# tky823/DNN-based_source_separation

Hardware: NVIDIA H100
Metric: audio-sec/s Conv-TasNet 2spk 4s@8kHz fwd+SI-SDR-PIT (higher is better)
Workload: dtype f32 via 3xFP16 split on wgmma (f16), fp32 accumulate

## Files before the change

dnn-based_source_separation_b200/csrc/ctn_wgmma.cu:

```cuda
#include "ctn_internal.h"
#include "ctn_wgmma_ptx.cuh"
#include "ctn_dw_math.cuh"
#include <cuda_fp16.h>
#include <stdlib.h>
#include <string.h>

int ctn_pw_simt(const PwArgs& a, int pro, int epi, cudaStream_t st);

namespace {

constexpr int TM = 128;
constexpr int KS = 32;
constexpr int NT = 128;
constexpr int THREADS = 256;
constexpr int CPW = 4;
constexpr int STAGES = 2;
constexpr int SMEM_HEADER = 1024;
constexpr int F16_MAX_ROWS = 2048;

template <int PRO, int EPI, bool F16>
__host__ __device__ constexpr bool chan_split() { return F16 && (PRO == PRO_DW || EPI == EPI_H); }
template <int PRO, int EPI, bool F16>
__host__ __device__ constexpr int tile_frames() { return chan_split<PRO, EPI, F16>() ? 64 : TM; }

struct TcArgs {
  PwArgs a;
  const float* wimg;
  const float* oscale;
  int n_tiles, k_slabs, t_tiles;
  int n_groups;
  int nt_per_cta;
};

template <int PRO>
__host__ __device__ constexpr int raw_q() { return PRO == PRO_DW ? 3 : PRO == PRO_RES ? 2 : 1; }
template <int PRO, int CPT>
struct Raw { float4 q[CPT][raw_q<PRO>()]; };

template <int PRO, int CPT>
__device__ __forceinline__ void load_raw(const PwArgs& a, int b, int c0, int tbase, int first, int step, bool interior, Raw<PRO, CPT>& r) {
#pragma unroll
  for (int j = 0; j < CPT; ++j) {
    const int c = c0 + j;
    if constexpr (PRO == PRO_DW) {
      const int cc = interior ? c : (c < a.K ? c : a.K - 1);
      const float* hr = a.A + ((size_t)b * a.K + cc) * a.pitch;
#pragma unroll
      for (int k = 0; k < 3; ++k) {
        int ts = first + k * step;
        if (!interior) ts = ts < 0 ? 0 : (ts > a.pitch - 4 ? a.pitch - 4 : ts);
        r.q[j][k] = __ldg(reinterpret_cast<const float4*>(hr + ts));
      }
    } else {
      const bool ok = c < a.K;
      r.q[j][0] = ok ? __ldg(reinterpret_cast<const float4*>(a.A + ((size_t)b * a.K + c) * a.pitch + tbase)) : make_float4(0.f, 0.f, 0.f, 0.f);
      if constexpr (PRO == PRO_RES)
        r.q[j][1] = ok ? __ldg(reinterpret_cast<const float4*>(a.res_r + ((size_t)b * a.res_Mt + c) * a.pitch + tbase))
                       : make_float4(0.f, 0.f, 0.f, 0.f);
    }
  }
}

template <int DCLS, bool INTERIOR, bool TRAIN, int CPT>
__device__ __forceinline__ void dw_form(const PwArgs& a, int b, int c0, int tbase, int first, int step, float2 mr1, float pslope,
                                        bool store_side, Raw<PRO_DW, CPT>& r, float4 (&v)[CPT], float2& dls, float2& dlss) {
  const float islope = TRAIN ? __ldg(a.dw_in_slope) : 0.f;
#pragma unroll
  for (int j = 0; j < CPT; ++j) {
    const int c = c0 + j;
    const int cc = INTERIOR ? c : (c < a.K ? c : a.K - 1);
    float4* q = r.q[j];
    if (TRAIN) {
#pragma unroll
      for (int k = 0; k < 3; ++k) {
        q[k].x = prelu_f(q[k].x, islope); q[k].y = prelu_f(q[k].y, islope); q[k].z = prelu_f(q[k].z, islope); q[k].w = prelu_f(q[k].w, islope);
      }
    }
    const float pg = __ldg(a.dw_norm_g + cc), pb = __ldg(a.dw_norm_b + cc), pbd = __ldg(a.dw_b + cc);
    const float w0 = __ldg(a.dw_w + cc * 3), w1 = __ldg(a.dw_w + cc * 3 + 1), w2 = __ldg(a.dw_w + cc * 3 + 2);
    const float gsc = pg * mr1.y, gsh = pb - mr1.x * mr1.y * pg;
    float4 pre;
    v[j] = dw_channel<DCLS, INTERIOR, TRAIN>(q[0], q[1], q[2], gsc, gsh, w0, w1, w2, pbd, pslope, first, step, tbase, a.frames, c < a.K,
                                             dls, dlss, &pre);
    if (TRAIN && store_side && c < a.K) *reinterpret_cast<float4*>(a.dw_u_pre_out + ((size_t)b * a.K + c) * a.pitch + tbase) = pre;
  }
}

template <int PRO, int EPI, int NPASS, bool F16, bool TRAIN>
__global__ void __launch_bounds__(THREADS, F16 ? 2 : 1) k_pw_wgmma(const TcArgs g) {
  constexpr bool CSPLIT = chan_split<PRO, EPI, F16>();
  constexpr int TMC = tile_frames<PRO, EPI, F16>();
  constexpr int NWG = CSPLIT ? 2 : 1;
  constexpr int LPR = TMC / 4;
  constexpr int CPT = CPW * LPR / 32;
  constexpr int NPREC = NPASS == 3 ? 2 : 1;
  constexpr uint32_t ROWB = F16 ? 64u : 128u;
  constexpr uint32_t A_BYTES = TMC * ROWB, W_BYTES = NT * ROWB;
  constexpr uint32_t STAGE_BYTES = NPREC * (A_BYTES + NWG * W_BYTES);
  static_assert(F16 || CPT == CPW, "the K-major tf32 store takes a warp's 4 channels per time step");
  extern __shared__ uint8_t smem_raw[];
  const uint32_t raw = ptx::smem_u32(smem_raw);
  const uint32_t base = (raw + 1023u) & ~1023u;
  uint8_t* smem = smem_raw + (base - raw);
  uint64_t* wbar = reinterpret_cast<uint64_t*>(smem);
  const uint32_t stage0 = base + SMEM_HEADER;
  const int warp = threadIdx.x >> 5, lane = threadIdx.x & 31, wg = warp >> 2;
  const PwArgs& a = g.a;

  const int n_groups = g.n_groups;
  const int ngrp = (int)blockIdx.x % n_groups;
  const int tt = ((int)blockIdx.x / n_groups) % g.t_tiles;
  const int b = (int)blockIdx.x / (n_groups * g.t_tiles);
  float* dacc = reinterpret_cast<float*>(smem + SMEM_HEADER + STAGES * STAGE_BYTES);

  if (threadIdx.x == 0) {
    for (int s = 0; s < STAGES; ++s) ptx::mbar_init(ptx::smem_u32(&wbar[s]), 1);
    ptx::fence_mbar_init();
  }
  __syncthreads();

  float act_s = 1.f;
  if (F16 && a.act_scale) act_s = __ldg(a.act_scale);
  float pslope = 0.f;
  if (PRO == PRO_PRELU || PRO == PRO_DW) pslope = __ldg(a.pro_slope);
  const int c_thr = warp * CPW + (lane / LPR) * CPT;
  const int tbase = tt * TMC + (lane % LPR) * 4;
  float2 mr1 = make_float2(0.f, 1.f), mr_res = make_float2(0.f, 1.f);
  if (PRO == PRO_DW) mr1 = gln_mean_rstd(a.dw_stats_in + 2 * b, (double)a.K * (double)a.frames, a.dw_eps);
  if (PRO == PRO_RES) mr_res = gln_mean_rstd(a.res_stats + 2 * b, a.res_n, a.res_eps);
  int dcls = 4, first = tbase, step = 0;
  bool dw_interior = false;
  if (PRO == PRO_DW) {
    const int d = a.dw_dilation;
    dcls = d >= 4 ? 4 : d;
    step = dcls == 4 ? d : 4;
    first = dcls == 4 ? tbase - a.dw_pad_left : tbase - 4;
    const int reach = d >= 4 ? d : 4;
    dw_interior = (tt * TMC - reach >= 0) && (tt * TMC + TMC - 1 + reach + 3 < a.frames) && (a.K % KS == 0) && (a.dw_pad_left == d);
  }
  if (EPI == EPI_MASKDEC)
    for (int i = threadIdx.x; i < TM * 16; i += THREADS) dacc[i] = 0.f;

  for (int ntl = 0; ntl < g.nt_per_cta; ++ntl) {
  const int nt0 = CSPLIT ? 2 * ngrp : ngrp * g.nt_per_cta + ntl;
  const int nt = CSPLIT ? nt0 + wg : nt0;
  const bool wg_live = nt < g.n_tiles;
  const int nw = CSPLIT ? min(2, g.n_tiles - nt0) : 1;
  const bool store_side = nt0 == 0;
  const uint8_t* wsrc = reinterpret_cast<const uint8_t*>(g.wimg) + (size_t)nt0 * g.k_slabs * NPREC * W_BYTES;
  float2 dls = make_float2(0.f, 0.f), dlss = make_float2(0.f, 0.f);
  float acc[64];
#pragma unroll
  for (int i = 0; i < 64; ++i) acc[i] = 0.f;

  Raw<PRO, CPT> cur;
  load_raw<PRO, CPT>(a, b, c_thr, tbase, first, step, dw_interior, cur);
  for (int ks = 0; ks < g.k_slabs; ++ks) {
    const int gk = ntl * g.k_slabs + ks;
    const int s = gk & 1;
    const uint32_t st_base = stage0 + (uint32_t)s * STAGE_BYTES;
    if (threadIdx.x == 0) {
      const uint32_t fb = ptx::smem_u32(&wbar[s]);
      ptx::mbar_arrive_expect_tx(fb, (uint32_t)nw * NPREC * W_BYTES);
      for (int w = 0; w < nw; ++w)
        ptx::bulk_g2s(st_base + NPREC * (A_BYTES + w * W_BYTES), wsrc + ((size_t)w * g.k_slabs + ks) * NPREC * W_BYTES, NPREC * W_BYTES, fb);
    }
    const int c0 = ks * KS + c_thr;
    float4 v[CPT];
    if constexpr (PRO == PRO_DW) {
      if (dw_interior) {
        if (dcls == 4) dw_form<4, true, TRAIN>(a, b, c0, tbase, first, step, mr1, pslope, store_side, cur, v, dls, dlss);
        else if (dcls == 2) dw_form<2, true, TRAIN>(a, b, c0, tbase, first, step, mr1, pslope, store_side, cur, v, dls, dlss);
        else dw_form<1, true, TRAIN>(a, b, c0, tbase, first, step, mr1, pslope, store_side, cur, v, dls, dlss);
      } else {
        if (dcls == 4) dw_form<4, false, TRAIN>(a, b, c0, tbase, first, step, mr1, pslope, store_side, cur, v, dls, dlss);
        else if (dcls == 2) dw_form<2, false, TRAIN>(a, b, c0, tbase, first, step, mr1, pslope, store_side, cur, v, dls, dlss);
        else dw_form<1, false, TRAIN>(a, b, c0, tbase, first, step, mr1, pslope, store_side, cur, v, dls, dlss);
      }
    } else {
#pragma unroll
      for (int j = 0; j < CPT; ++j) v[j] = cur.q[j][0];
      if (PRO == PRO_RES) {
#pragma unroll
        for (int j = 0; j < CPT; ++j) {
          const int k = c0 + j;
          const int kc = k < a.K ? k : a.K - 1;
          const float4 r = cur.q[j][PRO == PRO_RES ? 1 : 0];
          const float cst = __ldg(a.res_v1 + kc) - mr_res.x * mr_res.y * __ldg(a.res_v2 + kc);
          float4 xn;
          xn.x = fmaf(mr_res.y, r.x, v[j].x + cst); xn.y = fmaf(mr_res.y, r.y, v[j].y + cst);
          xn.z = fmaf(mr_res.y, r.z, v[j].z + cst); xn.w = fmaf(mr_res.y, r.w, v[j].w + cst);
          if (tbase + 0 >= a.frames) xn.x = 0.f;
          if (tbase + 1 >= a.frames) xn.y = 0.f;
          if (tbase + 2 >= a.frames) xn.z = 0.f;
          if (tbase + 3 >= a.frames) xn.w = 0.f;
          if (k >= a.K) xn = make_float4(0.f, 0.f, 0.f, 0.f);
          v[j] = xn;
          if (store_side && k < a.K) *reinterpret_cast<float4*>(a.res_x_out + ((size_t)b * a.K + k) * a.pitch + tbase) = xn;
        }
      }
      if (PRO == PRO_PRELU) {
#pragma unroll
        for (int j = 0; j < CPT; ++j) {
          v[j].x = prelu_f(v[j].x, pslope); v[j].y = prelu_f(v[j].y, pslope);
          v[j].z = prelu_f(v[j].z, pslope); v[j].w = prelu_f(v[j].w, pslope);
        }
      }
    }
    if (ks + 1 < g.k_slabs) load_raw<PRO, CPT>(a, b, (ks + 1) * KS + c_thr, tbase, first, step, dw_interior, cur);
    uint8_t* sa = smem + SMEM_HEADER + (size_t)s * STAGE_BYTES;
    if (F16) {
      const uint32_t f = (uint32_t)(tbase - tt * TMC);
#pragma unroll
      for (int j = 0; j < CPT; ++j) {
        const uint32_t c = (uint32_t)(c_thr + j);
        const uint32_t off = (f >> 6) * 4096u + (c >> 3) * 1024u + (c & 7) * 128u + ((((f >> 3) & 7) ^ (c & 7)) << 4) + (f & 7) * 2u;
        uint2 h2, l2;
        ptx::split_f16x2(v[j].x * act_s, v[j].y * act_s, h2.x, l2.x);
        ptx::split_f16x2(v[j].z * act_s, v[j].w * act_s, h2.y, l2.y);
        *reinterpret_cast<uint2*>(sa + off) = h2;
        *reinterpret_cast<uint2*>(sa + A_BYTES + off) = l2;
      }
    } else {
#pragma unroll
      for (int e = 0; e < 4; ++e) {
        const int t = lane * 4 + e;
        float x[CPW];
#pragma unroll
        for (int j = 0; j < CPW; ++j) x[j] = e == 0 ? v[j].x : e == 1 ? v[j].y : e == 2 ? v[j].z : v[j].w;
        const uint32_t off = (uint32_t)t * 128u + (((uint32_t)warp ^ (uint32_t)(t & 7)) << 4);
        float4 hi, lo;
        hi.x = ptx::hi_tf32(x[0]); hi.y = ptx::hi_tf32(x[1]); hi.z = ptx::hi_tf32(x[2]); hi.w = ptx::hi_tf32(x[3]);
        lo.x = x[0] - hi.x; lo.y = x[1] - hi.y; lo.z = x[2] - hi.z; lo.w = x[3] - hi.w;
        *reinterpret_cast<float4*>(sa + off) = hi;
        if (NPASS == 3) *reinterpret_cast<float4*>(sa + A_BYTES + off) = lo;
      }
    }
    ptx::fence_proxy_async_smem();
    __syncthreads();
    ptx::mbar_wait(ptx::smem_u32(&wbar[s]), (uint32_t)(gk >> 1) & 1u);
    if (wg_live) {
      const uint32_t a_hi = st_base + (CSPLIT ? 0u : (uint32_t)wg * 64u * ROWB), a_lo = a_hi + A_BYTES;
      const uint32_t w_hi = st_base + NPREC * (A_BYTES + (CSPLIT ? (uint32_t)wg * W_BYTES : 0u)), w_lo = w_hi + W_BYTES;
      ptx::wg_fence();
#pragma unroll
      for (int kk = 0; kk < (F16 ? KS / 16 : KS / 8); ++kk) {
        if (F16) {
          const uint64_t dah = ptx::wg_desc_mn128(a_hi + kk * 2048, 4096u, 1024u), dwh = ptx::wg_desc(w_hi + kk * 32, 8 * ROWB, ptx::SW64);
          ptx::wg_mma_f16(acc, dah, dwh);
          if (NPASS == 3) {
            const uint64_t dal = ptx::wg_desc_mn128(a_lo + kk * 2048, 4096u, 1024u), dwl = ptx::wg_desc(w_lo + kk * 32, 8 * ROWB, ptx::SW64);
            ptx::wg_mma_f16(acc, dal, dwh);
            ptx::wg_mma_f16(acc, dah, dwl);
          }
        } else {
          const uint64_t dah = ptx::wg_desc(a_hi + kk * 32, 8 * ROWB, ptx::SW128), dwh = ptx::wg_desc(w_hi + kk * 32, 8 * ROWB, ptx::SW128);
          ptx::wg_mma_tf32(acc, dah, dwh);
          if (NPASS == 3) {
            const uint64_t dal = ptx::wg_desc(a_lo + kk * 32, 8 * ROWB, ptx::SW128), dwl = ptx::wg_desc(w_lo + kk * 32, 8 * ROWB, ptx::SW128);
            ptx::wg_mma_tf32(acc, dal, dwh);
            ptx::wg_mma_tf32(acc, dah, dwl);
          }
        }
      }
      ptx::wg_commit();
      ptx::wg_wait<1>();
    }
    __syncthreads();
  }
  ptx::wg_wait<0>();

  if (PRO == PRO_DW && store_side) {
    const double sd = warp_sum_d((double)dls.x + (double)dls.y), ssd = warp_sum_d((double)dlss.x + (double)dlss.y);
    if (lane == 0) { atomicAdd(&a.dw_stats_out[2 * b], sd); atomicAdd(&a.dw_stats_out[2 * b + 1], ssd); }
  }
  if (!wg_live) continue;
  int n0 = nt * NT;
  asm volatile("" : "+r"(n0));

  float eslope = 0.f;
  if (EPI == EPI_H) eslope = __ldg(a.slope);
  const bool store_pre = EPI == EPI_H && a.store_pre != 0;
  float2 mr = make_float2(0.f, 1.f);
  if (EPI == EPI_HEAD) mr = gln_mean_rstd(a.stats_in + 2 * b, a.n_in, a.eps);
  const float inv_act = 1.f / act_s;
  const int row0 = (CSPLIT ? 0 : wg * 64) + (warp & 3) * 16 + (lane >> 2);
  float ls = 0.f, lss = 0.f;
  float dpart[2][16];
#pragma unroll
  for (int k = 0; k < 32; ++k) dpart[k >> 4][k & 15] = 0.f;
#pragma unroll
  for (int i = 0; i < 64; ++i) {
    const int row = row0 + 8 * ((i >> 1) & 1);
    const int n = n0 + 8 * (i >> 2) + 2 * (lane & 3) + (i & 1);
    const int t = tt * TMC + row;
    if (n >= a.M) continue;
    const bool tvalid = t < a.frames;
    const float osc = F16 ? __ldg(g.oscale + n) * inv_act : 1.f;
    float v = acc[i];
    float* q = a.D + ((size_t)b * a.M + n) * a.pitch + t;
    if (EPI == EPI_RAW) {
      if (F16) v *= osc;
    } else if (EPI == EPI_HEAD) {
      const float pv = __ldg(a.v1 + n) - mr.x * mr.y * __ldg(a.v2 + n);
      v = F16 ? fmaf(mr.y * osc, v, pv) : fmaf(mr.y, v, pv);
    } else if (EPI == EPI_H) {
      const float pre = F16 ? fmaf(v, osc, __ldg(a.bias + n)) : v + __ldg(a.bias + n);
      const float act = prelu_f(pre, eslope);
      v = store_pre ? pre : act;
      if (tvalid) { ls += act; lss = fmaf(act, act, lss); }
    } else if (EPI == EPI_MASK) {
      const float logit = F16 ? fmaf(v, osc, __ldg(a.bias + n)) : v + __ldg(a.bias + n);
      float mk;
      if (a.mask_logits) {
        mk = logit;
        v = logit;
      } else {
        mk = __fdividef(1.f, 1.f + __expf(-logit));
        v = tvalid ? mk * __ldg(a.wenc + ((size_t)b * a.Nb + n % a.Nb) * a.pitch + t) : 0.f;
      }
      if (a.mask_out) a.mask_out[((size_t)b * a.M + n) * a.pitch + t] = tvalid ? mk : 0.f;
    } else if (EPI == EPI_MASKDEC) {
      const float logit = F16 ? fmaf(v, osc, __ldg(a.bias + n)) : v + __ldg(a.bias + n);
      const float o = tvalid ? __fdividef(__ldg(a.wenc + ((size_t)b * a.Nb + n % a.Nb) * a.pitch + t), 1.f + __expf(-logit)) : 0.f;
      const float4* dr = reinterpret_cast<const float4*>(a.dec_w + (size_t)(n % a.Nb) * 16);
#pragma unroll
      for (int q4 = 0; q4 < 4; ++q4) {
        const float4 d4 = __ldg(dr + q4);
        float* dp = dpart[(i >> 1) & 1] + 4 * q4;
        dp[0] = fmaf(o, d4.x, dp[0]); dp[1] = fmaf(o, d4.y, dp[1]); dp[2] = fmaf(o, d4.z, dp[2]); dp[3] = fmaf(o, d4.w, dp[3]);
      }
      continue;
    }
    *q = tvalid ? v : 0.f;
  }
  if (EPI == EPI_H) {
    const double s = warp_sum_d((double)ls), ss = warp_sum_d((double)lss);
    if (lane == 0) { atomicAdd(&a.stats_out[2 * b], s); atomicAdd(&a.stats_out[2 * b + 1], ss); }
  }
  if (EPI == EPI_MASKDEC) {
#pragma unroll
    for (int k = 0; k < 32; ++k) {
      float v = dpart[k >> 4][k & 15];
      v += __shfl_xor_sync(0xffffffffu, v, 1);
      v += __shfl_xor_sync(0xffffffffu, v, 2);
      dpart[k >> 4][k & 15] = v;
    }
    if ((lane & 3) == 0) {
#pragma unroll
      for (int k = 0; k < 32; ++k) dacc[(row0 + 8 * (k >> 4)) * 16 + (k & 15)] += dpart[k >> 4][k & 15];
    }
  }
  }

  if (EPI == EPI_MASKDEC) {
    __syncthreads();
    const int src = ngrp, S = a.M / a.Nb;
    float* yo = a.D + ((size_t)b * S + src) * (size_t)a.dec_T_out;
    const long long base = 8LL * tt * TM - a.dec_crop_left;
    for (int sidx = threadIdx.x; sidx < 8 * TM + 8; sidx += THREADS) {
      const int f = sidx >> 3, k = sidx & 7;
      float v = 0.f;
      if (f < TM) v += dacc[f * 16 + k];
      if (f >= 1) v += dacc[(f - 1) * 16 + 8 + k];
      const long long tau = base + sidx;
      if (tau < 0 || tau >= a.dec_T_out) continue;
      if (sidx < 8 || sidx >= 8 * TM) atomicAdd(yo + tau, v);
      else yo[tau] = v;
    }
  }
}

__host__ __device__ __forceinline__ int wimg_offset(int nl, int kl) {
  return (nl >> 3) * 256 + (nl & 7) * 32 + ((((kl >> 2) ^ (nl & 7)) << 2) | (kl & 3));
}

__device__ __forceinline__ void wimg_f16_group(const float* __restrict__ W, int M, int K, int n_tile, int k_slabs, int nt, int grp,
                                               __half* __restrict__ img, float* __restrict__ oscale, float* smax) {
  static_assert(KS == 32, "one lane per channel of a slab");
  const int lane = threadIdx.x & 31, wid = threadIdx.x >> 5;
  const int nl = grp * 16 + wid;
  const int n = nt * n_tile + nl;
  const bool live = nl < n_tile && n < M;
  const float* row = W + (size_t)n * K;
  float mx = 0.f;
  if (live)
    for (int k = lane; k < K; k += 32) mx = fmaxf(mx, fabsf(row[k]));
#pragma unroll
  for (int o = 16; o > 0; o >>= 1) mx = fmaxf(mx, __shfl_xor_sync(0xffffffffu, mx, o));
  if (lane == 0) smax[wid] = mx;
  __syncthreads();
  mx = smax[lane & 15];
#pragma unroll
  for (int o = 8; o > 0; o >>= 1) mx = fmaxf(mx, __shfl_xor_sync(0xffffffffu, mx, o));
  __syncthreads();
  int e = 0;
  if (mx > 0.f && mx < INFINITY) e = 9 - ilogbf(mx);
  e = max(-100, min(100, e));
  const float up = ldexpf(1.f, e), down = ldexpf(1.f, -e);
  if (nl >= n_tile) return;
  if (lane == 0) oscale[n] = down;
  const size_t per = (size_t)n_tile * KS;
  for (int ks = 0; ks < k_slabs; ++ks) {
    const int kl = lane, k = ks * KS + kl;
    const float x = (live && k < K) ? row[k] * up : 0.f;
    __half* dst = img + ((size_t)nt * k_slabs + ks) * 2 * per;
    const int off = (nl >> 3) * 256 + (nl & 7) * 32 + ((((kl >> 3) ^ ((nl >> 1) & 3))) << 3) + (kl & 7);
    const __half hi = __float2half_rn(x);
    dst[off] = hi;
    dst[per + off] = __float2half_rn(x - __half2float(hi));
  }
}
__host__ __device__ inline size_t wimg_f16_image_bytes(int n_tile, int n_tiles, int k_slabs) {
  return (size_t)n_tiles * k_slabs * 2 * n_tile * KS * sizeof(__half);
}

struct WimgJobs { WimgJob j[CTN_MAX_JOBS]; };
__device__ __forceinline__ void wimg_tf32_slab(const float* __restrict__ W, int M, int K, int k_slabs, int nt, int ks, int nprec,
                                               float* __restrict__ wimg) {
  const int n_tile = NT;
  const size_t per = (size_t)n_tile * KS;
  float* dst = wimg + ((size_t)nt * k_slabs + ks) * nprec * per;
  for (int i = threadIdx.x; i < n_tile * KS; i += 256) {
    const int nl = i / KS, kl = i % KS;
    const int n = nt * n_tile + nl, k = ks * KS + kl;
    const float x = (n < M && k < K) ? W[(size_t)n * K + k] : 0.f;
    const int off = wimg_offset(nl, kl);
    const float hi = ptx::to_tf32(x);
    dst[off] = hi;
    if (nprec == 2) dst[per + off] = ptx::to_tf32(x - hi);
  }
}

__global__ void __launch_bounds__(256) k_build_wimg_batch(const WimgJobs jobs, int nprec) {
  const WimgJob& jb = jobs.j[blockIdx.y];
  const int n_tiles = (jb.M + NT - 1) / NT, k_slabs = (jb.K + KS - 1) / KS;
  const int blk = blockIdx.x;
  if (blk >= n_tiles * k_slabs) return;
  const int nt = blk / k_slabs, ks = blk - nt * k_slabs;
  wimg_tf32_slab(jb.W, jb.M, jb.K, k_slabs, nt, ks, nprec, jb.wimg);
}

__global__ void __launch_bounds__(512) k_build_wimg_batch_f16(const WimgJobs jobs) {
  __shared__ float smax[16];
  const WimgJob& jb = jobs.j[blockIdx.y];
  const int n_tile = NT;
  const int n_tiles = (jb.M + n_tile - 1) / n_tile, k_slabs = (jb.K + KS - 1) / KS;
  const int groups = n_tile / 16;
  __half* img = reinterpret_cast<__half*>(jb.wimg);
  float* oscale = reinterpret_cast<float*>(reinterpret_cast<uint8_t*>(jb.wimg) + wimg_f16_image_bytes(n_tile, n_tiles, k_slabs));
  for (int blk = blockIdx.x; blk < n_tiles * groups; blk += gridDim.x)
    wimg_f16_group(jb.W, jb.M, jb.K, n_tile, k_slabs, blk / groups, blk % groups, img, oscale, smax);
}

int eff_math(int M, int math) {
  if (math != CTN_MATH_F16X3) return math;
  return ((M + NT - 1) / NT) * NT > F16_MAX_ROWS ? CTN_MATH_TF32X3 : math;
}

template <int PRO, int EPI, int NPASS, bool F16, bool TRAIN>
int launch(const TcArgs& g0, cudaStream_t st) {
  constexpr int NPREC = NPASS == 3 ? 2 : 1;
  constexpr bool CSPLIT = chan_split<PRO, EPI, F16>();
  constexpr int TMC = tile_frames<PRO, EPI, F16>();
  constexpr size_t smem = SMEM_HEADER + 1024 + (size_t)STAGES * NPREC * (TMC + (CSPLIT ? 2 : 1) * NT) * (F16 ? 64 : 128) +
                          (EPI == EPI_MASKDEC ? TM * 16 * 4 : 0);
  TcArgs g = g0;
  g.t_tiles = g.a.pitch / TMC;
  g.n_groups = CSPLIT ? (g.n_tiles + 1) / 2 : g.n_tiles / g.nt_per_cta;
  static bool attr_done[CTN_MAX_DEVICES] = {false};
  const int dev = ctn_current_device();
  if (!attr_done[dev]) {
    cudaError_t e = cudaFuncSetAttribute(k_pw_wgmma<PRO, EPI, NPASS, F16, TRAIN>, cudaFuncAttributeMaxDynamicSharedMemorySize, (int)smem);
    if (e != cudaSuccess) return (int)e;
    attr_done[dev] = true;
  }
  const long long grid = (long long)g.a.B * g.t_tiles * g.n_groups;
  if (grid > 0x7fffffffLL) return CTN_EUNSUPPORTED;
  k_pw_wgmma<PRO, EPI, NPASS, F16, TRAIN><<<(unsigned)grid, THREADS, smem, st>>>(g);
  CTN_COUNT_LAUNCH();
  CTN_RETURN_IF_CUDA_ERR();
  return CTN_OK;
}

template <int PRO, int EPI, bool TRAIN = false>
int launch_math(const TcArgs& g, int math, cudaStream_t st) {
  if (math == CTN_MATH_F16X3) return launch<PRO, EPI, 3, true, TRAIN>(g, st);
  if (math == CTN_MATH_TF32) return launch<PRO, EPI, 1, false, TRAIN>(g, st);
  return launch<PRO, EPI, 3, false, TRAIN>(g, st);
}

int piece_math(int math, bool bounded) { return math == CTN_MATH_F16X3 && !bounded ? CTN_MATH_TF32X3 : math; }

int build_images(const WimgJob* jobs, int n, int math, cudaStream_t st) {
  const bool f16 = math == CTN_MATH_F16X3;
  for (int i0 = 0; i0 < n; i0 += CTN_MAX_JOBS) {
    WimgJobs wj;
    const int m = n - i0 < CTN_MAX_JOBS ? n - i0 : CTN_MAX_JOBS;
    int maxb = 1;
    for (int i = 0; i < m; ++i) {
      const WimgJob& jb = jobs[i0 + i];
      wj.j[i] = jb;
      const int blocks = ((jb.M + NT - 1) / NT) * (f16 ? NT / 16 : (jb.K + KS - 1) / KS);
      if (blocks > maxb) maxb = blocks;
    }
    if (f16) k_build_wimg_batch_f16<<<dim3(maxb, m), 512, 0, st>>>(wj);
    else k_build_wimg_batch<<<dim3(maxb, m), 256, 0, st>>>(wj, math == CTN_MATH_TF32 ? 1 : 2);
    CTN_COUNT_LAUNCH();
  }
  CTN_RETURN_IF_CUDA_ERR();
  return CTN_OK;
}

bool maskdec_ok(const PwArgs& a, int pmath) {
  return eff_math(a.M, pmath) == CTN_MATH_F16X3 && a.dec_w && a.Nb > 0 && a.Nb % NT == 0 && a.M % a.Nb == 0 &&
         (((uintptr_t)a.dec_w) & 15) == 0;
}

int launch_wgmma(const PwArgs& a, int pro, int epi, int pmath, cudaStream_t st) {
  if (!a.wimg) return CTN_EINVAL;
  const int math = eff_math(a.M, pmath);
  if (a.pitch % TM != 0) return CTN_EALIGN;
  if ((((uintptr_t)a.A) | ((uintptr_t)a.wimg)) & 15) return CTN_EALIGN;
  TcArgs g;
  g.a = a;
  g.wimg = a.wimg;
  g.n_tiles = (a.M + NT - 1) / NT;
  g.k_slabs = (a.K + KS - 1) / KS;
  g.oscale = math == CTN_MATH_F16X3
                 ? reinterpret_cast<const float*>(reinterpret_cast<const uint8_t*>(a.wimg) + wimg_f16_image_bytes(NT, g.n_tiles, g.k_slabs))
                 : nullptr;
  g.nt_per_cta = 1;
  const bool train_dw = pro == PRO_DW && a.dw_u_pre_out != nullptr;
  if (pro == PRO_NONE && epi == EPI_RAW) return launch_math<PRO_NONE, EPI_RAW>(g, math, st);
  if (pro == PRO_DW && epi == EPI_RAW)
    return train_dw ? launch_math<PRO_DW, EPI_RAW, true>(g, math, st) : launch_math<PRO_DW, EPI_RAW>(g, math, st);
  if (pro == PRO_NONE && epi == EPI_HEAD) return launch_math<PRO_NONE, EPI_HEAD>(g, math, st);
  if (pro == PRO_NONE && epi == EPI_H) return launch_math<PRO_NONE, EPI_H>(g, math, st);
  if (pro == PRO_RES && epi == EPI_H) return launch_math<PRO_RES, EPI_H>(g, math, st);
  if (pro == PRO_PRELU && epi == EPI_MASK) return launch_math<PRO_PRELU, EPI_MASK>(g, math, st);
  if (pro == PRO_PRELU && epi == EPI_MASKDEC) {
    if (!maskdec_ok(a, pmath)) return CTN_EUNSUPPORTED;
    g.nt_per_cta = a.Nb / NT;
    return launch<PRO_PRELU, EPI_MASKDEC, 3, true, false>(g, st);
  }
  return CTN_EUNSUPPORTED;
}

}

extern "C" int ctn_has_tcgen05(void) { return 1; }

size_t ctn_pw_wimg_bytes(int M, int K, int math) {
  const int nprec = math == CTN_MATH_TF32 ? 1 : 2;
  const int n_tiles = (M + NT - 1) / NT, k_slabs = (K + KS - 1) / KS;
  return (size_t)n_tiles * k_slabs * nprec * NT * KS * sizeof(float) + (size_t)n_tiles * NT * sizeof(float) + 256;
}

size_t ctn_pw_wimg_max_bytes(const int (*shapes)[2], int n, int math) {
  if (math == CTN_MATH_FP32) return 256;
  size_t mx = 0;
  for (int i = 0; i < n; ++i) {
    const size_t b = ctn_pw_wimg_bytes(shapes[i][0], shapes[i][1], math);
    if (b > mx) mx = b;
  }
  return mx;
}

int ctn_pw_prepare(const PwArgs& a, int math, float* wimg, cudaStream_t st) {
  const WimgJob job{a.W, wimg, a.M, a.K};
  return ctn_pw_prepare_batch(&job, 1, math, a.act_scale != nullptr, st);
}

int ctn_pw_prepare_batch(const WimgJob* jobs, int n, int math, bool bounded, cudaStream_t st) {
  if (math == CTN_MATH_FP32) return CTN_OK;
  math = piece_math(math, bounded);
  bool uniform = true;
  for (int i = 0; i < n; ++i) uniform = uniform && eff_math(jobs[i].M, math) == math;
  if (uniform) return build_images(jobs, n, math, st);
  for (int i = 0; i < n; ++i) CTN_TRY(build_images(jobs + i, 1, eff_math(jobs[i].M, math), st));
  return CTN_OK;
}

int ctn_pw_maskdec_supported(const PwArgs& a, int math) { return maskdec_ok(a, piece_math(math, a.act_scale != nullptr)); }

int ctn_pw(const PwArgs& a, int pro, int epi, int math, float* wimg_scratch, cudaStream_t st) {
  if (math == CTN_MATH_FP32) return ctn_pw_simt(a, pro, epi, st);
  const int pmath = piece_math(math, a.act_scale != nullptr);
  if (!wimg_scratch) return launch_wgmma(a, pro, epi, pmath, st);
  CTN_TRY(ctn_pw_prepare(a, math, wimg_scratch, st));
  PwArgs b = a;
  b.wimg = wimg_scratch;
  return launch_wgmma(b, pro, epi, pmath, st);
}
```

Baseline: 7404.

## Add dedicated mask-decoder kernel with resident activations and deep weight ring

```diff
diff --git a/dnn-based_source_separation_b200/csrc/ctn_wgmma.cu b/dnn-based_source_separation_b200/csrc/ctn_wgmma.cu
--- a/dnn-based_source_separation_b200/csrc/ctn_wgmma.cu
+++ b/dnn-based_source_separation_b200/csrc/ctn_wgmma.cu
@@ -111,7 +111,6 @@
   const int ngrp = (int)blockIdx.x % n_groups;
   const int tt = ((int)blockIdx.x / n_groups) % g.t_tiles;
   const int b = (int)blockIdx.x / (n_groups * g.t_tiles);
-  float* dacc = reinterpret_cast<float*>(smem + SMEM_HEADER + STAGES * STAGE_BYTES);
 
   if (threadIdx.x == 0) {
     for (int s = 0; s < STAGES; ++s) ptx::mbar_init(ptx::smem_u32(&wbar[s]), 1);
@@ -138,8 +137,6 @@
     const int reach = d >= 4 ? d : 4;
     dw_interior = (tt * TMC - reach >= 0) && (tt * TMC + TMC - 1 + reach + 3 < a.frames) && (a.K % KS == 0) && (a.dw_pad_left == d);
   }
-  if (EPI == EPI_MASKDEC)
-    for (int i = threadIdx.x; i < TM * 16; i += THREADS) dacc[i] = 0.f;
 
   for (int ntl = 0; ntl < g.nt_per_cta; ++ntl) {
   const int nt0 = CSPLIT ? 2 * ngrp : ngrp * g.nt_per_cta + ntl;
@@ -286,9 +283,6 @@
   const float inv_act = 1.f / act_s;
   const int row0 = (CSPLIT ? 0 : wg * 64) + (warp & 3) * 16 + (lane >> 2);
   float ls = 0.f, lss = 0.f;
-  float dpart[2][16];
-#pragma unroll
-  for (int k = 0; k < 32; ++k) dpart[k >> 4][k & 15] = 0.f;
 #pragma unroll
   for (int i = 0; i < 64; ++i) {
     const int row = row0 + 8 * ((i >> 1) & 1);
@@ -320,17 +314,6 @@
         v = tvalid ? mk * __ldg(a.wenc + ((size_t)b * a.Nb + n % a.Nb) * a.pitch + t) : 0.f;
       }
       if (a.mask_out) a.mask_out[((size_t)b * a.M + n) * a.pitch + t] = tvalid ? mk : 0.f;
-    } else if (EPI == EPI_MASKDEC) {
-      const float logit = F16 ? fmaf(v, osc, __ldg(a.bias + n)) : v + __ldg(a.bias + n);
-      const float o = tvalid ? __fdividef(__ldg(a.wenc + ((size_t)b * a.Nb + n % a.Nb) * a.pitch + t), 1.f + __expf(-logit)) : 0.f;
-      const float4* dr = reinterpret_cast<const float4*>(a.dec_w + (size_t)(n % a.Nb) * 16);
-#pragma unroll
-      for (int q4 = 0; q4 < 4; ++q4) {
-        const float4 d4 = __ldg(dr + q4);
-        float* dp = dpart[(i >> 1) & 1] + 4 * q4;
-        dp[0] = fmaf(o, d4.x, dp[0]); dp[1] = fmaf(o, d4.y, dp[1]); dp[2] = fmaf(o, d4.z, dp[2]); dp[3] = fmaf(o, d4.w, dp[3]);
-      }
-      continue;
     }
     *q = tvalid ? v : 0.f;
   }
@@ -338,35 +321,180 @@
     const double s = warp_sum_d((double)ls), ss = warp_sum_d((double)lss);
     if (lane == 0) { atomicAdd(&a.stats_out[2 * b], s); atomicAdd(&a.stats_out[2 * b + 1], ss); }
   }
-  if (EPI == EPI_MASKDEC) {
-#pragma unroll
-    for (int k = 0; k < 32; ++k) {
-      float v = dpart[k >> 4][k & 15];
-      v += __shfl_xor_sync(0xffffffffu, v, 1);
-      v += __shfl_xor_sync(0xffffffffu, v, 2);
-      dpart[k >> 4][k & 15] = v;
-    }
-    if ((lane & 3) == 0) {
-#pragma unroll
-      for (int k = 0; k < 32; ++k) dacc[(row0 + 8 * (k >> 4)) * 16 + (k & 15)] += dpart[k >> 4][k & 15];
-    }
-  }
-  }
-
-  if (EPI == EPI_MASKDEC) {
+  }
+}
+
+constexpr int MD_MAX_K = 128;
+constexpr int MD_STAGES = 4;
+constexpr int MD_ROW = 20;
+constexpr uint32_t MD_A_BYTES = TM * 64u, MD_W_BYTES = NT * 64u;
+constexpr int MD_TAB = NT * 16 + 2 * NT;
+constexpr size_t MD_SMEM = 1024 + SMEM_HEADER + (size_t)(MD_MAX_K / KS) * 2 * MD_A_BYTES + (size_t)MD_STAGES * 2 * MD_W_BYTES +
+                           (size_t)TM * MD_ROW * sizeof(float) + 2 * (size_t)MD_TAB * sizeof(float);
+
+__global__ void __launch_bounds__(THREADS, 1) k_maskdec(const TcArgs g) {
+  extern __shared__ uint8_t smem_raw[];
+  const uint32_t raw = ptx::smem_u32(smem_raw);
+  const uint32_t base = (raw + 1023u) & ~1023u;
+  uint8_t* smem = smem_raw + (base - raw);
+  uint64_t* wbar = reinterpret_cast<uint64_t*>(smem);
+  const uint32_t op0 = base + SMEM_HEADER;
+  const uint32_t ring0 = op0 + (uint32_t)(MD_MAX_K / KS) * 2 * MD_A_BYTES;
+  float* dacc = reinterpret_cast<float*>(smem + (ring0 - base) + MD_STAGES * 2 * MD_W_BYTES);
+  float* tab0 = dacc + TM * MD_ROW;
+  const int warp = threadIdx.x >> 5, lane = threadIdx.x & 31, wg = warp >> 2;
+  const PwArgs& a = g.a;
+  const int tt = (int)blockIdx.x % g.t_tiles, b = (int)blockIdx.x / g.t_tiles;
+  const int ntps = a.Nb / NT, n_tiles = g.n_tiles, k_slabs = g.k_slabs;
+  const int total = n_tiles * k_slabs;
+  const uint8_t* wimg = reinterpret_cast<const uint8_t*>(g.wimg);
+
+  for (int i = threadIdx.x; i < TM * MD_ROW; i += THREADS) dacc[i] = 0.f;
+  if (threadIdx.x == 0) {
+    for (int s = 0; s < MD_STAGES; ++s) ptx::mbar_init(ptx::smem_u32(&wbar[s]), 1);
+    ptx::fence_mbar_init();
+  }
+  __syncthreads();
+  int issued = 0;
+  auto refill = [&](int consumed) {
+    for (; issued < total && issued < consumed + MD_STAGES; ++issued) {
+      const uint32_t fb = ptx::smem_u32(&wbar[issued % MD_STAGES]);
+      ptx::mbar_arrive_expect_tx(fb, 2 * MD_W_BYTES);
+      ptx::bulk_g2s(ring0 + (uint32_t)(issued % MD_STAGES) * 2 * MD_W_BYTES, wimg + (size_t)issued * 2 * MD_W_BYTES, 2 * MD_W_BYTES, fb);
+    }
+  };
+  if (threadIdx.x == 0) refill(0);
+
+  const float act_s = __ldg(a.act_scale), pslope = __ldg(a.pro_slope);
+  {
+    const int tbase = tt * TM + lane * 4;
+    float4 v[MD_MAX_K / KS][CPW];
+#pragma unroll
+    for (int ks = 0; ks < MD_MAX_K / KS; ++ks)
+#pragma unroll
+      for (int j = 0; j < CPW; ++j) {
+        const int c = ks * KS + warp * CPW + j;
+        v[ks][j] = ks < k_slabs && c < a.K ? __ldg(reinterpret_cast<const float4*>(a.A + ((size_t)b * a.K + c) * a.pitch + tbase))
+                                           : make_float4(0.f, 0.f, 0.f, 0.f);
+      }
+    const uint32_t f = (uint32_t)lane * 4u;
+#pragma unroll
+    for (int ks = 0; ks < MD_MAX_K / KS; ++ks) {
+      if (ks >= k_slabs) break;
+      uint8_t* sa = smem + (op0 - base) + (size_t)ks * 2 * MD_A_BYTES;
+#pragma unroll
+      for (int j = 0; j < CPW; ++j) {
+        float4 x = v[ks][j];
+        x.x = prelu_f(x.x, pslope); x.y = prelu_f(x.y, pslope); x.z = prelu_f(x.z, pslope); x.w = prelu_f(x.w, pslope);
+        const uint32_t c = (uint32_t)(warp * CPW + j);
+        const uint32_t off = (f >> 6) * 4096u + (c >> 3) * 1024u + (c & 7) * 128u + ((((f >> 3) & 7) ^ (c & 7)) << 4) + (f & 7) * 2u;
+        uint2 h2, l2;
+        ptx::split_f16x2(x.x * act_s, x.y * act_s, h2.x, l2.x);
+        ptx::split_f16x2(x.z * act_s, x.w * act_s, h2.y, l2.y);
+        *reinterpret_cast<uint2*>(sa + off) = h2;
+        *reinterpret_cast<uint2*>(sa + MD_A_BYTES + off) = l2;
+      }
+    }
+  }
+  ptx::fence_proxy_async_smem();
+  __syncthreads();
+
+  const float inv_act = 1.f / act_s;
+  const int row0 = wg * 64 + (warp & 3) * 16 + (lane >> 2);
+  const int t0 = tt * TM + row0;
+  const int S = a.M / a.Nb;
+  for (int nt = 0; nt < n_tiles; ++nt) {
+    const int src = nt / ntps, nb0 = (nt - src * ntps) * NT;
+    float wv[64];
+    {
+      const float* wr = a.wenc + ((size_t)b * a.Nb + nb0 + 2 * (lane & 3)) * a.pitch + t0;
+#pragma unroll
+      for (int i = 0; i < 64; ++i) wv[i] = __ldg(wr + (size_t)(8 * (i >> 2) + (i & 1)) * a.pitch + 8 * ((i >> 1) & 1));
+    }
+    const int tc = threadIdx.x & (NT - 1), th = threadIdx.x >> 7;
+    const float4* dsrc = reinterpret_cast<const float4*>(a.dec_w + (size_t)(nb0 + tc) * 16) + 2 * th;
+    const float4 td0 = __ldg(dsrc), td1 = __ldg(dsrc + 1);
+    const float tsb = th == 0 ? __ldg(g.oscale + nt * NT + tc) * inv_act : __ldg(a.bias + nt * NT + tc);
+    float acc[64];
+#pragma unroll
+    for (int i = 0; i < 64; ++i) acc[i] = 0.f;
+    for (int ks = 0; ks < k_slabs; ++ks) {
+      const int q = nt * k_slabs + ks;
+      const uint32_t w_hi = ring0 + (uint32_t)(q % MD_STAGES) * 2 * MD_W_BYTES, w_lo = w_hi + MD_W_BYTES;
+      const uint32_t a_hi = op0 + (uint32_t)ks * 2 * MD_A_BYTES + (uint32_t)wg * 4096u, a_lo = a_hi + MD_A_BYTES;
+      ptx::mbar_wait(ptx::smem_u32(&wbar[q % MD_STAGES]), (uint32_t)(q / MD_STAGES) & 1u);
+      ptx::wg_fence();
+#pragma unroll
+      for (int kk = 0; kk < KS / 16; ++kk) {
+        const uint64_t dah = ptx::wg_desc_mn128(a_hi + kk * 2048, 4096u, 1024u), dwh = ptx::wg_desc(w_hi + kk * 32, 8 * 64, ptx::SW64);
+        const uint64_t dal = ptx::wg_desc_mn128(a_lo + kk * 2048, 4096u, 1024u), dwl = ptx::wg_desc(w_lo + kk * 32, 8 * 64, ptx::SW64);
+        ptx::wg_mma_f16(acc, dah, dwh);
+        ptx::wg_mma_f16(acc, dal, dwh);
+        ptx::wg_mma_f16(acc, dah, dwl);
+      }
+      ptx::wg_commit();
+    }
+    ptx::wg_wait<0>();
+    float* tab = tab0 + (nt & 1) * MD_TAB;
+    float4* tdec = reinterpret_cast<float4*>(tab);
+    tdec[(2 * th) * NT + tc] = td0;
+    tdec[(2 * th + 1) * NT + tc] = td1;
+    tab[NT * 16 + th * NT + tc] = tsb;
     __syncthreads();
-    const int src = ngrp, S = a.M / a.Nb;
-    float* yo = a.D + ((size_t)b * S + src) * (size_t)a.dec_T_out;
-    const long long base = 8LL * tt * TM - a.dec_crop_left;
-    for (int sidx = threadIdx.x; sidx < 8 * TM + 8; sidx += THREADS) {
-      const int f = sidx >> 3, k = sidx & 7;
-      float v = 0.f;
-      if (f < TM) v += dacc[f * 16 + k];
-      if (f >= 1) v += dacc[(f - 1) * 16 + 8 + k];
-      const long long tau = base + sidx;
-      if (tau < 0 || tau >= a.dec_T_out) continue;
-      if (sidx < 8 || sidx >= 8 * TM) atomicAdd(yo + tau, v);
-      else yo[tau] = v;
+    if (threadIdx.x == 0) refill((nt + 1) * k_slabs);
+
+    float dpart[2][16];
+#pragma unroll
+    for (int k = 0; k < 32; ++k) dpart[k >> 4][k & 15] = 0.f;
+#pragma unroll
+    for (int i = 0; i < 64; ++i) {
+      const int c = 8 * (i >> 2) + 2 * (lane & 3) + (i & 1);
+      const bool tvalid = t0 + 8 * ((i >> 1) & 1) < a.frames;
+      const float osc = tab[NT * 16 + c];
+      const float logit = fmaf(acc[i], osc, tab[NT * 17 + c]);
+      const float o = tvalid ? __fdividef(wv[i], 1.f + __expf(-logit)) : 0.f;
+#pragma unroll
+      for (int q4 = 0; q4 < 4; ++q4) {
+        const float4 d4 = tdec[q4 * NT + c];
+        float* dp = dpart[(i >> 1) & 1] + 4 * q4;
+        dp[0] = fmaf(o, d4.x, dp[0]); dp[1] = fmaf(o, d4.y, dp[1]); dp[2] = fmaf(o, d4.z, dp[2]); dp[3] = fmaf(o, d4.w, dp[3]);
+      }
+    }
+    const bool hb0 = lane & 1, hb1 = lane & 2;
+    float r1[16];
+#pragma unroll
+    for (int j = 0; j < 16; ++j) {
+      const float keep = hb0 ? dpart[1][j] : dpart[0][j], send = hb0 ? dpart[0][j] : dpart[1][j];
+      r1[j] = keep + __shfl_xor_sync(0xffffffffu, send, 1);
+    }
+    float r2[8];
+#pragma unroll
+    for (int j = 0; j < 8; ++j) {
+      const float keep = hb1 ? r1[8 + j] : r1[j], send = hb1 ? r1[j] : r1[8 + j];
+      r2[j] = keep + __shfl_xor_sync(0xffffffffu, send, 2);
+    }
+    float4* dst = reinterpret_cast<float4*>(dacc + (row0 + (hb0 ? 8 : 0)) * MD_ROW + (hb1 ? 8 : 0));
+    float4 u0 = dst[0], u1 = dst[1];
+    u0.x += r2[0]; u0.y += r2[1]; u0.z += r2[2]; u0.w += r2[3];
+    u1.x += r2[4]; u1.y += r2[5]; u1.z += r2[6]; u1.w += r2[7];
+    dst[0] = u0; dst[1] = u1;
+
+    if (nt - src * ntps == ntps - 1) {
+      __syncthreads();
+      float* yo = a.D + ((size_t)b * S + src) * (size_t)a.dec_T_out;
+      const long long tb = 8LL * tt * TM - a.dec_crop_left;
+      for (int j = threadIdx.x; j < 2 * 32 * (TM / 8 + 1); j += THREADS) {
+        const int u = j >> 5, f = (u >> 1) * 8 + 2 * ((j & 31) >> 3) + (u & 1), k = j & 7;
+        if (f > TM) continue;
+        const int sidx = 8 * f + k;
+        float v = 0.f;
+        if (f < TM) { v += dacc[f * MD_ROW + k]; dacc[f * MD_ROW + k] = 0.f; }
+        if (f >= 1) { v += dacc[(f - 1) * MD_ROW + 8 + k]; dacc[(f - 1) * MD_ROW + 8 + k] = 0.f; }
+        const long long tau = tb + sidx;
+        if (tau < 0 || tau >= a.dec_T_out) continue;
+        if (sidx < 8 || sidx >= 8 * TM) atomicAdd(yo + tau, v);
+        else yo[tau] = v;
+      }
     }
   }
 }
@@ -463,8 +591,7 @@
   constexpr int NPREC = NPASS == 3 ? 2 : 1;
   constexpr bool CSPLIT = chan_split<PRO, EPI, F16>();
   constexpr int TMC = tile_frames<PRO, EPI, F16>();
-  constexpr size_t smem = SMEM_HEADER + 1024 + (size_t)STAGES * NPREC * (TMC + (CSPLIT ? 2 : 1) * NT) * (F16 ? 64 : 128) +
-                          (EPI == EPI_MASKDEC ? TM * 16 * 4 : 0);
+  constexpr size_t smem = SMEM_HEADER + 1024 + (size_t)STAGES * NPREC * (TMC + (CSPLIT ? 2 : 1) * NT) * (F16 ? 64 : 128);
   TcArgs g = g0;
   g.t_tiles = g.a.pitch / TMC;
   g.n_groups = CSPLIT ? (g.n_tiles + 1) / 2 : g.n_tiles / g.nt_per_cta;
@@ -513,8 +640,27 @@
 }
 
 bool maskdec_ok(const PwArgs& a, int pmath) {
-  return eff_math(a.M, pmath) == CTN_MATH_F16X3 && a.dec_w && a.Nb > 0 && a.Nb % NT == 0 && a.M % a.Nb == 0 &&
+  return eff_math(a.M, pmath) == CTN_MATH_F16X3 && a.dec_w && a.Nb > 0 && a.Nb % NT == 0 && a.M % a.Nb == 0 && a.K <= MD_MAX_K &&
          (((uintptr_t)a.dec_w) & 15) == 0;
+}
+
+int launch_maskdec(const TcArgs& g0, cudaStream_t st) {
+  TcArgs g = g0;
+  g.t_tiles = g.a.pitch / TM;
+  g.n_groups = 1;
+  static bool attr_done[CTN_MAX_DEVICES] = {false};
+  const int dev = ctn_current_device();
+  if (!attr_done[dev]) {
+    cudaError_t e = cudaFuncSetAttribute(k_maskdec, cudaFuncAttributeMaxDynamicSharedMemorySize, (int)MD_SMEM);
+    if (e != cudaSuccess) return (int)e;
+    attr_done[dev] = true;
+  }
+  const long long grid = (long long)g.a.B * g.t_tiles;
+  if (grid > 0x7fffffffLL) return CTN_EUNSUPPORTED;
+  k_maskdec<<<(unsigned)grid, THREADS, MD_SMEM, st>>>(g);
+  CTN_COUNT_LAUNCH();
+  CTN_RETURN_IF_CUDA_ERR();
+  return CTN_OK;
 }
 
 int launch_wgmma(const PwArgs& a, int pro, int epi, int pmath, cudaStream_t st) {
@@ -541,8 +687,7 @@
   if (pro == PRO_PRELU && epi == EPI_MASK) return launch_math<PRO_PRELU, EPI_MASK>(g, math, st);
   if (pro == PRO_PRELU && epi == EPI_MASKDEC) {
     if (!maskdec_ok(a, pmath)) return CTN_EUNSUPPORTED;
-    g.nt_per_cta = a.Nb / NT;
-    return launch<PRO_PRELU, EPI_MASKDEC, 3, true, false>(g, st);
+    return launch_maskdec(g, st);
   }
   return CTN_EUNSUPPORTED;
 }
```

Result: faster. 7822 (median of 6 runs) (+5.6%).
